# tavildar/Polar

Measured on AMD Instinct MI355X. Metric: codewords/s (N=2048 K=1024 L=32 LLR-SCL), higher is better.
Workload: dtype f64

## Files before the change

polar_amd/build.py:

```python
import os
import shutil
import subprocess
import sys

HERE = os.path.dirname(os.path.abspath(__file__))
ROOT = os.path.dirname(HERE)
CSRC = os.path.join(HERE, "csrc")
INC = os.path.join(ROOT, "include")
LIB = os.path.join(HERE, "libpolar_amd.so")
BUILD = os.path.join(HERE, "_build")
FLAGS_LIST32 = ["-mllvm", "-amdgpu-sched-strategy=max-memory-clause", "-mllvm", "-amdgpu-use-amdgpu-trackers"] + \
               os.environ.get("POLAR_LIST32_FLAGS", "").split()
FLAGS_LAT = os.environ.get("POLAR_LAT_FLAGS", "").split()
SOURCES = [("polar_kernels.hip", ["POLAR_ED_TU=0"], "", []), ("polar_kernels.hip", ["POLAR_ED_TU=1"], ".ed", []),
           ("polar_kernels.hip", ["POLAR_ED_TU=2"], ".ed32", FLAGS_LIST32), ("polar_kernels.hip", ["POLAR_ED_TU=3"], ".lat", FLAGS_LAT),
           ("polar_kernels.hip", ["POLAR_ED_TU=4"], ".list", []),
           ("polar_kernels.hip", ["POLAR_ED_TU=5"], ".headA", []), ("polar_kernels.hip", ["POLAR_ED_TU=6"], ".headB", FLAGS_LIST32),
           ("polar_kernels.hip", ["POLAR_ED_TU=7"], ".adapt", []),
           ("polar_kernels_sc.hip", [], "", []), ("polar_kernels_p1.hip", [], "", []), ("polar_channel.hip", [], "", []),
           ("polar_construct.hip", [], "", []), ("polar_kernels_mlc.hip", [], "", []), ("polar_kernels_ga.hip", [], "", []),
           ("polar_kernels_metric.hip", [], "", []), ("polar_kernels_adapt.hip", [], "", []),
           ("polar_kernels_flip.hip", [], "", [])] + \
          [(f, [], "", []) for f in ("polar_handle.cpp", "polar_decode.cpp", "polar_hostpipe.cpp", "polar_montecarlo.cpp", "polar_multi.cpp",
                                     "polar_debug.cpp", "polar_ga.cpp", "polar_bicm.cpp", "polar_list.cpp", "polar_mlc.cpp", "polar_adaptive.cpp", "polar_flip.cpp")]
TEST_HOOK_SOURCES = ("polar_montecarlo.cpp", "polar_debug.cpp")
TEST_HOOK_KERNEL_TAGS = (".ed32", ".headB")
LIB_TEST = os.path.join(HERE, "libpolar_amd_test.so")
KNOWN_DEFS = {"POLAR_MARGIN", "POLAR_SLOTHIST", "SCLAT_PROF", "POLAR_DEV_GS32", "POLAR_DEV_ONE", "POLAR_NO_FIXED_N",
              "POLAR_NO_GUARD_INT", "POLAR_NO_COLD_HINTS", "OCC", "ED_NR"}
ARCH = os.environ.get("POLAR_ARCH", "gfx950")
_flags_ok = {}


def _probe_flags(flags):
    key = tuple(flags)
    if key not in _flags_ok:
        import tempfile
        ok = list(flags)
        with tempfile.TemporaryDirectory() as d:
            src = os.path.join(d, "probe.hip")
            open(src, "w").write("#include <hip/hip_runtime.h>\n__global__ void probe_kernel() {}\n")
            pairs = [flags[i:i + 2] for i in range(0, len(flags), 2)]
            ok = []
            for pr in pairs:
                r = subprocess.run([_hipcc(), "--offload-arch=" + ARCH, "-c", src, "-o", os.path.join(d, "probe.o")] + pr,
                                   stdout=subprocess.DEVNULL, stderr=subprocess.PIPE, text=True)
                if r.returncode == 0 or "Unknown command line argument" not in r.stderr:
                    ok += pr
                else:
                    print("polar_amd.build: this compiler rejects %s (%s); building without it" %
                          (" ".join(pr), (r.stderr.strip().splitlines() or ["?"])[-1][:120]), file=sys.stderr)
        _flags_ok[key] = ok
    return _flags_ok[key]


def _hipcc():
    return shutil.which("hipcc") or "/opt/rocm/bin/hipcc"


def _torch_lib():
    try:
        import torch
        d = os.path.join(os.path.dirname(torch.__file__), "lib")
        if os.path.exists(os.path.join(d, "libamdhip64.so")):
            return d
    except Exception:
        pass
    return None


def _newer(target, deps):
    if not os.path.exists(target):
        return True
    t = os.path.getmtime(target)
    return any((not os.path.exists(d)) or os.path.getmtime(d) > t for d in deps)


def _fingerprint(cmd, files):
    import hashlib
    root = os.path.realpath(ROOT)

    def rel(x):
# ... 133 lines not shown
```

polar_amd/csrc/polar_debug.cpp:

```cpp
#include "polar_multi.h"
#include "polar_amd_debug.h"
#ifdef POLAR_TEST_HOOKS
#include "polar_head_plan.h"
hipError_t polar_r1_counts_read_ed32(unsigned long long *out);
hipError_t polar_r1_counts_read_head(unsigned long long *out);
#endif

extern "C" {

int polar_debug_weak_leaves(const polar_code_t *h) { return polar_get_weak_leaves(h); }

int polar_debug_set(polar_code_t *h, const char *key, long value) {
    if (!h || !key) return fail(POLAR_E_ARG, "NULL argument");
    polar_code::Knobs &k = h->knobs;
    const std::string s(key);
    if (s == "mode_override") { if (value < -1 || value > 2) return fail(POLAR_E_ARG, "mode_override must be -1 (none), 0, 1 or 2"); k.mode_override = (int)value; }
    else if (s == "sc_no_fold") k.sc_no_fold = value != 0;
    else if (s == "no_tables") k.no_tables = value != 0;
    else if (s == "no_head") k.no_head = value != 0;
    else if (s == "no_r1") k.no_r1 = value != 0;
    else if (s == "head_min_b") { if (value < 0) return fail(POLAR_E_ARG, "head_min_b must be >= 0 (0 = default)"); k.head_min_b = value; }
    else if (s == "no_fuse_front") k.no_fuse_front = value != 0;
    else if (s == "no_prefix") h->prefix_on = (value == 0);
    else if (s == "no_rccl") { k.no_rccl = value != 0; multi_release(h, false); }
// ... 13 lines not shown
    else if (s == "host_lanes") { if (value < 0 || value > HostPipe::kMaxLanes) return fail(POLAR_E_ARG, "host_lanes must be 0 (default) or 1 .. %d", HostPipe::kMaxLanes); k.host_lanes = value; }
    else if (s == "host_ramp") k.host_ramp = value;
    else if (s == "host_prefault") { if (value < -1 || value > 16) return fail(POLAR_E_ARG, "host_prefault must be -1 (none), 0 (default) or 1 .. 16 threads"); k.host_prefault = value; }
    else if (s == "host_threads") { if (value < 0) return fail(POLAR_E_ARG, "host_threads must be >= 0"); k.host_threads = value; }
    else if (s == "multi_grace_s") { if (value < 0) return fail(POLAR_E_ARG, "multi_grace_s must be >= 0"); k.multi_grace_s = value; }
#ifdef POLAR_TEST_HOOKS
    else if (s == "force_workers") { k.force_workers = value != 0; multi_release(h, false); }
    else if (s == "stall_device") k.stall_device = (int)value;
    else if (s == "stall_ms") { if (value < 0) return fail(POLAR_E_ARG, "stall_ms must be >= 0"); k.stall_ms = value; }
#endif
    else if (s == "multi_timeout_s") { if (value < 0) return fail(POLAR_E_ARG, "multi_timeout_s must be >= 0 (0 = no watchdog)"); k.multi_timeout_s = value; }
    else return fail(POLAR_E_ARG, "polar_debug_set: unknown key '%s'", key);
    drop_clones(h);
    return POLAR_OK;
}
void *polar_debug_scratch_ptr(polar_code_t *h) { return h ? (void *)h->d_llr_scr.p : nullptr; }
long polar_debug_get(const polar_code_t *h, const char *key) {
    if (!key) return -1;
    const std::string s(key);
    if (s == "allocs") return (long)g_allocs.load();
    if (s == "comm_inits") return (long)polar_debug_comm_inits();
    if (!h) return -1;
    if (s == "test_hooks") {
#ifdef POLAR_TEST_HOOKS
        return 1;
#else
        return 0;
#endif
    }
    if (s == "weak_leaves") return h->weak_leaves;
    if (s == "mode_override") return h->knobs.mode_override;
    if (s == "head_phi") return h->last_head_phi;
    if (s == "lat_waves") return h->last_lat_waves;
    if (s == "lane_waves") return h->last_lane_waves;
#ifdef POLAR_TEST_HOOKS
    if (s == "head_check") {
        if (!h->last_head_phi || h->last_head_b <= 0 || !h->d_head_rec.p) return -2;
        int P = 0;
        while (P < h->N && h->frozen[P]) ++P;
        const int Q = P >= 256 ? 256 : (P < 33 ? 0 : (P < 64 ? 64 : (P < 128 ? 128 : 256)));
        const HeadPlan hp = head_plan(h->frozen.data(), h->n, Q, std::min(P, Q), h->N / 2);
        if (hp.phi_h != h->last_head_phi) return -3;
        std::vector<unsigned long long> rows2((size_t)h->last_head_b * 4);
        const size_t pitch = hp.record_words() * sizeof(unsigned long long);
        if (hipMemcpy2D(rows2.data(), 32, h->d_head_rec.p + 2 * 4, pitch, 32, (size_t)h->last_head_b, hipMemcpyDeviceToHost) != hipSuccess) return -4;
        long bad = 0;
        for (long b = 0; b < h->last_head_b; ++b) {
            unsigned long long r[4];
            for (int a = 0; a < 4; ++a) r[a] = rows2[(size_t)b * 4 + a];
            bad += head_record_ok(hp, r) ? 0 : 1;
        }
        return bad;
    }
    if (s == "r1_committed" || s == "r1_discarded") {
        unsigned long long c[2] = {0, 0};
        if ((h->last_head_phi ? polar_r1_counts_read_head(c) : polar_r1_counts_read_ed32(c)) != hipSuccess) return -2;
        return (long)c[s == "r1_discarded" ? 1 : 0];
    }
#endif
    if (s == "last_rounds") return h->last_rounds;
    if (s == "last_round_max_per_device") return h->last_round_max_per_device;
    if (s == "worker_threads_started") return h->worker_threads_started;
    if (s.compare(0, 9, "round_us_") == 0) {
        if (h->round_us.empty()) return 0;
        std::vector<long> v(h->round_us);
        if (s == "round_us_count") return (long)v.size();
        if (s == "round_us_first") return v.front();
        std::sort(v.begin(), v.end());
        if (s == "round_us_min") return v.front();
        if (s == "round_us_max") return v.back();
        if (s == "round_us_median") return v[v.size() / 2];
        return -1;
    }
    if (s == "multi_poisoned") return h->multi_poisoned ? 1 : 0;
    if (s == "host_chunks") return h->hpipe ? h->hpipe->last_chunks : 0;
    if (s == "host_chunk_cw") return h->hpipe ? h->hpipe->last_chunk_cw : 0;
    if (s == "host_lanes") return h->hpipe ? h->hpipe->last_lanes : 0;
    if (s == "host_threads") return h->hpipe ? h->hpipe->last_threads : 0;
    if (s == "host_us_copy_in") return h->hpipe ? h->hpipe->us_copy_in : 0;
    if (s == "host_us_wait") return h->hpipe ? h->hpipe->us_wait : 0;
    if (s == "host_us_copy_out") return h->hpipe ? h->hpipe->us_copy_out : 0;
    if (s == "host_us_total") return h->hpipe ? h->hpipe->us_total : 0;
    return -1;
}
int polar_debug_comm_inits(void) { return g_comm_inits.load(); }

long polar_debug_fallback_rows(polar_code_t *h, uint32_t *rows, long cap) {
    if (!h || !h->fb_count) return -1;
    DevGuard dg_;
    if (ensure_device(h, dg_)) return -1;
    hipError_t e = hipStreamSynchronize((hipStream_t)h->fb_stream);
    unsigned int count = 0;
    if (e == hipSuccess) e = hipMemcpy(&count, h->fb_count, sizeof count, hipMemcpyDeviceToHost);
    if (e == hipSuccess && (long)count > h->fb_b) return -(long)hipErrorInvalidValue - 1;
    const long n = std::min<long>(count, cap);
    if (e == hipSuccess && rows && n > 0) e = hipMemcpy(rows, h->fb_list, (size_t)n * sizeof(uint32_t), hipMemcpyDeviceToHost);
    return e == hipSuccess ? (long)count : -(long)e - 1;
}

long polar_debug_ctl_words(polar_code_t *h, uint32_t *words, long cap, int marked) {
    if (!h) return -1;
    DevGuard dg_;
    if (ensure_device(h, dg_)) return -1;
    const long n = std::min<long>(h->N, cap);
    if (words && n > 0) {
        const hipError_t e = hipMemcpy(words, marked ? h->d_ctl_r1.p : h->d_ctl.p, (size_t)n * sizeof(uint32_t), hipMemcpyDeviceToHost);
        if (e != hipSuccess) return -(long)e - 1;
    }
    return h->N;
}
// ... 3 lines not shown
```

polar_amd/csrc/polar_kernels.hip:

```cpp
#include <hip/hip_runtime.h>
#include <stdint.h>
#include <type_traits>

#include "polar_kernels.h"
#include "polar_device.h"
#include "polar_edom.h"

#ifdef POLAR_PROFILE
#define PROF_DECL u64 prof_acc[32] = {0,0,0,0,0,0,0,0,0,0,0,0,0,0,0,0,0,0,0,0,0,0,0,0,0,0,0,0,0,0,0,0}; u64 prof_t = __builtin_readcyclecounter();
#define PROF(i) { u64 t_ = __builtin_readcyclecounter(); prof_acc[i] += t_ - prof_t; prof_t = t_; }
#define PROF_OUT if (lane == 0 && p.pm_out) { for (int i_ = 0; i_ < 32; ++i_) atomicAdd((u64 *)p.pm_out + i_, prof_acc[i_]); }
#define PROF_CNT(i, v) { prof_acc[i] += (u64)(v); }
#define PROF_HEAD_DECL const int prof_head_phi = p.pm_out ? (int)((const u64 *)p.pm_out)[32] : 0; const u64 prof_head_t0 = prof_t; bool prof_head_open = prof_head_phi > 0;
#define PROF_HEAD(phi_) if (prof_head_open && (phi_) >= prof_head_phi) { prof_acc[22] += __builtin_readcyclecounter() - prof_head_t0; prof_head_open = false; }
#define PROF_HEAD_END prof_acc[23] += __builtin_readcyclecounter() - prof_head_t0;
#define PROF_R1_DECL int prof_r1_left = 0; bool prof_r1_open = false; u64 prof_r1_t0 = 0; const bool prof_r1_off = p.pm_out && ((const u64 *)p.pm_out)[33] != 0; (void)prof_r1_off;
#define PROF_R1_TOP { if (prof_r1_open) { prof_acc[24] += prof_t - prof_r1_t0; prof_r1_open = false; } \
                      if (prof_r1_left > 0) { prof_r1_t0 = prof_t; prof_r1_open = true; --prof_r1_left; } }
#define PROF_R1_LEAF(ctl_, fast_) { const int rb_ = (int)((ctl_) >> 9) & 3; \
                      if (prof_r1_open) { if (!(fast_)) prof_acc[27] += 1; } \
                      else if (rb_) { if (fast_) { prof_acc[25] += 1; prof_r1_left = (1 << rb_) - 1; } else prof_acc[26] += 1; } }
#define PROF_R1_COMMIT prof_r1_left = 0;
#define PROF_R1_END if (prof_r1_open) { prof_acc[24] += __builtin_readcyclecounter() - prof_r1_t0; prof_r1_open = false; }
#else
#define PROF_R1_DECL constexpr bool prof_r1_off = false; (void)prof_r1_off;
#define PROF_R1_TOP
#define PROF_R1_LEAF(ctl_, fast_)
#define PROF_R1_COMMIT
#define PROF_R1_END
#define PROF_HEAD_DECL
#define PROF_HEAD(phi_)
#define PROF_HEAD_END
#define PROF_DECL
#define PROF(i)
#define PROF_CNT(i, v)
#define PROF_OUT
#endif

#include "polar_llr_nodes.h"

template <bool NARROW16>
__device__ __forceinline__ const double *ch_row(const PolarDecodeParams &p, size_t cw, int N) {
    if constexpr (NARROW16) {
        if (p.llr_fmt >= POLAR_LLR_F16) return reinterpret_cast<const double *>(reinterpret_cast<const uint16_t *>(p.llr) + cw * (size_t)N);
    }
    return p.llr_fmt ? reinterpret_cast<const double *>(reinterpret_cast<const float *>(p.llr) + cw * (size_t)N)
                     : p.llr + cw * (size_t)N;
}
template <bool NARROW16>
__device__ __forceinline__ double ch_narrow(const double *row, size_t i, int fmt) {
    if constexpr (NARROW16) return llr_load_narrow(row, i, fmt);
    else return (double)reinterpret_cast<const float *>(row)[i];
}
#define CH(row, i) (p.llr_fmt ? ch_narrow<CH_N16>(row, i, p.llr_fmt) : (row)[i])

#ifndef FU
#define FU 4
#endif
#ifndef POLAR_SKIP_L1
#define POLAR_SKIP_L1 1
#endif
#define POLAR_SADDR 1
#ifndef OCC
#define OCC 4
#endif
#define LANE_CTX                                   \
    const int lane = LAT ? lane_k : lane_id_opaque();    \
    const int lig = lane & (GS - 1);               \
    const int gbase = lane & ~(GS - 1);            \
    (void)lig; (void)gbase;
#if defined(POLAR_ED_TU) && POLAR_ED_TU == 4
#define POLAR_LIST_OUT 1
#define scl_decode_llr_kernel scl_decode_llr_list_kernel
#define POLAR_KPARAMS PolarListParams
#elif defined(POLAR_ED_TU) && POLAR_ED_TU == 7
#define POLAR_ADAPT_OUT 1
#define scl_decode_llr_kernel scl_decode_llr_adapt_kernel
#define POLAR_KPARAMS PolarAdaptParams
#elif defined(POLAR_ED_TU) && (POLAR_ED_TU == 5 || POLAR_ED_TU == 6)
#define POLAR_HEAD (POLAR_ED_TU == 5 ? 1 : 2)
#define scl_decode_llr_kernel scl_decode_llr_head_kernel
#define POLAR_KPARAMS PolarHeadParams
#else
#define POLAR_KPARAMS PolarDecodeParams
#endif
#ifndef POLAR_HEAD
#define POLAR_HEAD 0
#endif
#if defined(POLAR_ED_TU) && (POLAR_ED_TU == 2 || POLAR_ED_TU == 6) && !defined(POLAR_MARGIN)
#define POLAR_R1 1
#else
#define POLAR_R1 0
#endif
#if POLAR_R1 && defined(POLAR_TEST_HOOKS)
__device__ unsigned long long polar_r1_counts_dev[2];
#define R1_CNT_DECL unsigned r1_cnt_c = 0, r1_cnt_d = 0;
#define R1_CNT_COMMIT ++r1_cnt_c;
#define R1_CNT_DISCARD ++r1_cnt_d;
#define R1_CNT_OUT if (lane == 0) { atomicAdd(&polar_r1_counts_dev[0], (unsigned long long)r1_cnt_c); atomicAdd(&polar_r1_counts_dev[1], (unsigned long long)r1_cnt_d); }
#else
#define R1_CNT_DECL
#define R1_CNT_COMMIT
#define R1_CNT_DISCARD
#define R1_CNT_OUT
#endif
template <int GS, int LDS_LOG, int PIPE, bool ED, int NL = 0, int LAT = 0>
__global__ __launch_bounds__(PIPE ? 64 : 256, PIPE ? 2 : OCC) void scl_decode_llr_kernel(POLAR_KPARAMS p) {
    constexpr int WPB = PIPE ? 1 : 4;
    constexpr bool CH_N16 = !ED;
    constexpr int G = LAT ? 1 : 64 / GS;
    constexpr int EL = 64 / GS;
    constexpr int CST = LAT ? GS : 64;
#define POLAR_CL (LAT ? lig : lane)
#define POLAR_CGB (LAT ? 0 : gbase)
    constexpr int SL = 1 << LDS_LOG;
    const int lane = threadIdx.x & 63;
    const int wib = __builtin_amdgcn_readfirstlane((int)(threadIdx.x >> 6));
    const int wave_id = blockIdx.x * WPB + wib;
    const int nwaves = gridDim.x * WPB;
    const int lane_k = lane;
    (void)lane_k;
    const int lig = lane & (GS - 1);
    const int gbase = lane & ~(GS - 1);
    const int grp = LAT ? 0 : lane / GS;
    const int n = NL ? NL : p.n, N = NL ? (1 << NL) : p.N, K = p.K, L = p.L;
    const u64 gmask = (GS == 64) ? ~0ull : ((1ull << GS) - 1ull);

    extern __shared__ __attribute__((aligned(16))) unsigned char smem[];
    double *tabs = reinterpret_cast<double *>(smem);
    constexpr size_t WAVE_LDS = (size_t)(2 * SL - 1) * 64 * 8 + 128 * 8 + 128;
    unsigned char *wbase = smem + 324 * 8 + (size_t)wib * WAVE_LDS;
    double *lds_llr = reinterpret_cast<double *>(wbase);
    double *sortbuf = lds_llr + (LAT ? 0 : (size_t)(2 * SL - 1) * 64);
    unsigned char *stackv = reinterpret_cast<unsigned char *>(sortbuf + 128);
    unsigned char *srcof = stackv + 64;
    for (int i = threadIdx.x; i < 322; i += WPB * 64) tabs[i] = p.tabs[i];
    if (WPB > 1) __syncthreads();
    const Tabs tb = {tabs, tabs + 64, tabs + 64 + 129};
    u64 guard = 0;
    double gacc = __builtin_inf();
    auto FN = [&](double a, double b) -> double {
        if constexpr (ED) return f_node_e_acc(a, b, gacc); else return f_node(a, b, tb);
    };
    auto GN = [&](double a, double b, uint32_t cw_, int bi) -> double {
        if constexpr (ED) return g_node_e(a, b, cw_ << (31 - bi), tb); else return g_node(a, b, (cw_ >> bi) & 1u);
    };
    const long Bv = p.cw_count ? (long)*p.cw_count : (p.n_dev ? ((long)*p.n_dev < p.B ? (long)*p.n_dev : p.B) : p.B);

    const size_t big_elems = (N > 2 * SL) ? (size_t)(N - 2 * SL) : 0;
    double *g_llr = LAT ? nullptr : p.llr_scr + (size_t)wave_id * big_elems * 64;
    const int cwords = (N >= 128) ? (N / 32 - 2) : 0;
    double *lat_ch = reinterpret_cast<double *>(stackv + 128);
    double *lat_a = lat_ch + N;
    uint32_t *lat_w = reinterpret_cast<uint32_t *>(lat_a + (size_t)N * GS);
    uint32_t *g_cl = LAT ? lat_w : p.c_scr + (size_t)wave_id * 2 * (size_t)cwords * 64;
    uint32_t *g_cr = g_cl + (size_t)cwords * CST;
// ... 604 lines not shown
}
#elif POLAR_ED_TU == 0
hipError_t polar_launch_decode_lat_ed1(const PolarDecodeParams &p, int gs, int blocks, hipStream_t st);
hipError_t polar_launch_decode_lat(const PolarDecodeParams &p, int gs, bool ed, int blocks, hipStream_t st) {
    if (ed) return polar_launch_decode_lat_ed1(p, gs, blocks, st);
    if (gs == 2) return launch_lat<2, false>(p, blocks, st);
    return hipErrorInvalidValue;
}
size_t polar_decode_lat_lds_bytes(int N, int gs, int W) {
    return 324 * 8 + (128 * 8 + 128) + (size_t)N * 8 + (size_t)N * gs * 8 + (2 * polar_decode_cwords(N) + (size_t)3 * W) * gs * 4 + 64;
}
#endif

#if POLAR_ED_TU == 4 || POLAR_ED_TU == 7
template <int GS>
static hipError_t launch_finish(const POLAR_KPARAMS &p, int grid, hipStream_t st) {
    const int wpb = polar_decode_waves_per_block(0);
    const size_t lds = polar_decode_lds_bytes(3, 0);
    hipLaunchKernelGGL((scl_decode_llr_kernel<GS, 3, 0, false>), dim3(grid / wpb), dim3(64 * wpb), lds, st, p);
    return hipGetLastError();
}
static hipError_t launch_finish_gs(const POLAR_KPARAMS &p, int gs, int grid, hipStream_t st) {
    switch (gs) {
        case 1: return launch_finish<1>(p, grid, st);
        case 2: return launch_finish<2>(p, grid, st);
        case 4: return launch_finish<4>(p, grid, st);
        case 8: return launch_finish<8>(p, grid, st);
        case 16: return launch_finish<16>(p, grid, st);
        case 32: return launch_finish<32>(p, grid, st);
        case 64: return launch_finish<64>(p, grid, st);
        default: return hipErrorInvalidValue;
    }
}
#if POLAR_ED_TU == 4
hipError_t polar_launch_decode_llr_list(const PolarListParams &p, int gs, int grid, hipStream_t st) {
    if (!p.list_cand || grid < 4 || (grid & 3)) return hipErrorInvalidValue;
    return launch_finish_gs(p, gs, grid, st);
}
#else
hipError_t polar_launch_decode_llr_adapt(const PolarAdaptParams &p, int gs, int grid, hipStream_t st) {
    if (!p.out || !p.ad_retry || grid < 4 || (grid & 3)) return hipErrorInvalidValue;
    return launch_finish_gs(p, gs, grid, st);
}
#endif
#elif POLAR_ED_TU == 5
hipError_t polar_launch_decode_head_export(const PolarHeadParams &p, int grid, hipStream_t st) {
    if (!p.head_rec || p.L != 4 || p.head_phi <= 0 || p.head_phi >= p.N || grid < 4 || (grid & 3)) return hipErrorInvalidValue;
    hipLaunchKernelGGL((scl_decode_llr_kernel<4, 3, 0, true>), dim3(grid / 4), dim3(256), polar_decode_lds_bytes(3, 0), st, p);
    return hipGetLastError();
}
#elif POLAR_ED_TU == 6
#ifdef POLAR_TEST_HOOKS
static hipError_t r1_counts_zero(hipStream_t st) {
    static const unsigned long long z[2] = {0, 0};
    return hipMemcpyToSymbolAsync(HIP_SYMBOL(polar_r1_counts_dev), z, sizeof z, 0, hipMemcpyHostToDevice, st);
}
hipError_t polar_r1_counts_read_head(unsigned long long *out) { return hipMemcpyFromSymbol(out, HIP_SYMBOL(polar_r1_counts_dev), 2 * sizeof(unsigned long long)); }
#endif
hipError_t polar_launch_decode_head_import(const PolarHeadParams &p, int grid, hipStream_t st) {
#ifdef POLAR_TEST_HOOKS
    if (hipError_t e = r1_counts_zero(st)) return e;
#endif
    if (!p.head_rec || p.L < 17 || p.L > 32 || p.head_phi <= 0 || p.head_phi >= p.N || grid < 4 || (grid & 3)) return hipErrorInvalidValue;
    const size_t lds = polar_decode_lds_bytes(3, 0);
#ifndef POLAR_NO_FIXED_N
    if (p.n == 11) hipLaunchKernelGGL((scl_decode_llr_kernel<32, 3, 0, true, 11>), dim3(grid / 4), dim3(256), lds, st, p);
    else if (p.n == 10) hipLaunchKernelGGL((scl_decode_llr_kernel<32, 3, 0, true, 10>), dim3(grid / 4), dim3(256), lds, st, p);
    else
#endif
    hipLaunchKernelGGL((scl_decode_llr_kernel<32, 3, 0, true>), dim3(grid / 4), dim3(256), lds, st, p);
    return hipGetLastError();
}
#elif POLAR_ED_TU == 2
#ifdef POLAR_TEST_HOOKS
hipError_t polar_r1_counts_read_ed32(unsigned long long *out) { return hipMemcpyFromSymbol(out, HIP_SYMBOL(polar_r1_counts_dev), 2 * sizeof(unsigned long long)); }
#endif
hipError_t polar_launch_decode_llr_ed1_gs32(const PolarDecodeParams &p, int lds_log, int pipe, int grid, hipStream_t st) {
#ifdef POLAR_TEST_HOOKS
    {
        static const unsigned long long z[2] = {0, 0};
        if (hipError_t e = hipMemcpyToSymbolAsync(HIP_SYMBOL(polar_r1_counts_dev), z, sizeof z, 0, hipMemcpyHostToDevice, st)) return e;
    }
#endif
    return launch_gs<32, true>(p, lds_log, pipe, grid, st);
}
#elif POLAR_ED_TU == 1
hipError_t polar_launch_decode_llr_ed1_gs32(const PolarDecodeParams &p, int lds_log, int pipe, int grid, hipStream_t st);
hipError_t polar_launch_decode_llr_ed1(const PolarDecodeParams &p, int gs, int lds_log, int pipe, int grid, hipStream_t st) {
    switch (gs) {
#ifndef POLAR_DEV_GS32
        case 4: return launch_gs<4, true>(p, lds_log, pipe, grid, st);
        case 8: return launch_gs<8, true>(p, lds_log, pipe, grid, st);
        case 16: return launch_gs<16, true>(p, lds_log, pipe, grid, st);
        case 64: return launch_gs<64, true>(p, lds_log, pipe, grid, st);
#endif
        case 32: return polar_launch_decode_llr_ed1_gs32(p, lds_log, pipe, grid, st);
        default: return hipErrorInvalidValue;
    }
}
#elif POLAR_ED_TU == 0
hipError_t polar_launch_decode_llr_ed0(const PolarDecodeParams &p, int gs, int lds_log, int pipe, int grid, hipStream_t st) {
    switch (gs) {
        case 1: return launch_gs<1, false>(p, lds_log, pipe, grid, st);
#ifndef POLAR_DEV_GS32
        case 2: return launch_gs<2, false>(p, lds_log, pipe, grid, st);
        case 4: return launch_gs<4, false>(p, lds_log, pipe, grid, st);
        case 8: return launch_gs<8, false>(p, lds_log, pipe, grid, st);
        case 16: return launch_gs<16, false>(p, lds_log, pipe, grid, st);
        case 64: return launch_gs<64, false>(p, lds_log, pipe, grid, st);
#endif
        case 32: return launch_gs<32, false>(p, lds_log, pipe, grid, st);
        default: return hipErrorInvalidValue;
    }
}
hipError_t polar_launch_decode_llr(const PolarDecodeParams &p, int gs, int lds_log, int pipe, int grid, bool ed, hipStream_t st) {
    return ed ? polar_launch_decode_llr_ed1(p, gs, lds_log, pipe, grid, st) : polar_launch_decode_llr_ed0(p, gs, lds_log, pipe, grid, st);
}
#endif
```

polar_amd/csrc/polar_scl_leaf.inc:

```
            if (zb) {
                const int Z = 1 << zb;
                LANE_CTX
                auto block4 = [&](double v0, double v1, double v2, double v3) {
                    double lf[4] = {0, 0, 0, 0};
                    if (active) {
                        double a0, a1;
                        FN2(v0, v2, v1, v3, a0, a1);
                        const double b0 = GN(v0, v2, 0u, 0), b1 = GN(v1, v3, 0u, 0);
                        FN2(a0, a1, b0, b1, lf[0], lf[2]);
                        lf[1] = GN(a0, a1, 0u, 0); lf[3] = GN(b0, b1, 0u, 0);
                    }
                    if constexpr (LAT && ED) {
                        bool ng[4]; double alz[4], sneg[4], spos[4];
                        leaf_terms_ed_block<4>(lf, actw, tb, ng, alz, sneg, spos);
#pragma unroll
                        for (int i = 0; i < 4; ++i)
                            if (active) pm += ng[i] ? spos[i] : sneg[i];
                    } else {
#pragma unroll
                    for (int i = 0; i < 4; ++i) {
                        bool ng; double alz, sneg, spos;
                        leaf_terms<ED>(lf[i], active, actw, tb, ng, alz, sneg, spos);
                        if (active) pm += ng ? spos : sneg;
                    }
// ... 36 lines not shown
                phi += Z - 1;
                continue;
            }
            LANE_CTX
            const u64 below = (1ull << lig) - 1ull;
            const bool frozen = (ctl & 1u) != 0;
            unsigned ubit = 0;
            if (frozen) {
                bool ng; double alz, sneg, spos;
                if constexpr (LAT && ED) {
                    const double lf1[1] = {leaf}; bool ng1[1]; double al1[1], sn1[1], sp1[1];
                    leaf_terms_ed_block<1>(lf1, actw, tb, ng1, al1, sn1, sp1);
                    ng = ng1[0]; alz = al1[0]; sneg = sn1[0]; spos = sp1[0];
                } else leaf_terms<ED>(leaf, active, actw, tb, ng, alz, sneg, spos);
                if (active) pm += ng ? spos : sneg;
            } else {
                const u64 actm = LAT ? (actw & gmask) : ((actw >> gbase) & gmask);
                const int nact = __popcll(actm);
                const int rho = (2 * nact < L) ? 2 * nact : L;
                bool lneg; double al;
                double gm = -__builtin_inf(), bl = __builtin_inf();
                double sneg, spos;
                if constexpr (LAT && ED) {
                    const double lf1[1] = {leaf}; bool ng1[1]; double al1[1], sn1[1], sp1[1];
                    leaf_terms_ed_block<1>(lf1, actw, tb, ng1, al1, sn1, sp1);
                    lneg = ng1[0]; al = al1[0]; sneg = sn1[0]; spos = sp1[0];
                } else leaf_terms<ED>(leaf, active, actw, tb, lneg, al, sneg, spos);
                if constexpr (ED) {
                    if (POLAR_UNLIKELY2(ctl & 0x100u)) guard |= __ballot(active && fabs(leaf) > 0.99999999 && fabs(leaf) <= 1.0);
                }
                if (active) {
                    gm = pm + sneg;
                    bl = (pm + al) * 0.99999999999909050530;
                }
                bool fast;
                {
                    unsigned gh = active ? (unsigned)__double2hiint(gm) : 0u;
                    unsigned bh = active ? (unsigned)__double2hiint(bl) : 0xFFFFFFFFu;
                    group_max_min_u32<GS>(gh, bh);
                    if constexpr (LAT) {
                        fast = (nact == 0) || (nact == L && ((__builtin_amdgcn_uicmp(gh, bh, 36) | ~group_result_rows<GS>()) == ~0ull));
                    } else {
                    const u64 m_ok = __builtin_amdgcn_sicmp(nact, 0, 32) | (__builtin_amdgcn_sicmp(nact, L, 32) & __builtin_amdgcn_uicmp(gh, bh, 36));
                    fast = ((m_ok | ~group_result_rows<GS>()) == ~0ull);
                    }
                }
                double gmax = 0.0;
                if (!fast) {
                    gmax = group_reduce<GS, true>(gm, lane);
                    const double bmin = group_reduce<GS, false>(bl, lane);
                    fast = wave_all((nact == 0) || (nact == L && gmax < bmin));
                }
                PROF_CNT(8, 1)
                PROF_R1_LEAF(ctl, fast)
                PROF(16)
                if (fast) {
                    PROF_CNT(9, 1)
#ifdef POLAR_MARGIN
                    {
                        const double gx = group_reduce<GS, true>(active ? gm : -__builtin_inf(), lane);
                        const double bx = group_reduce<GS, false>(active ? pm + spos : __builtin_inf(), lane);
                        if (nact == L) mingap = __builtin_fmin(mingap, bx - gx);
                    }
#endif
                    if (active) {
                        ubit = lneg ? 1u : 0u;
                        pm = gm;
                        hword |= ubit << (t & 31);
                    }
                    PROF(17)
#if POLAR_R1
                    if constexpr (ED && !LAT && GS == 32) {
                    if ((ctl & 0x600u) && !prof_r1_off) {
                        PROF_CNT(29, 1)
                        const uint32_t ctl_r1 = ctlp[phi + 4 < N ? phi + 4 : 0];
                        const double *yq = lds_llr + (size_t)1 * 64 + lane, *xq = lds_llr + (size_t)3 * 64 + lane;
                        double lf[3] = {0.0, 0.0, 0.0};
                        if (active) {
                            const double y0 = yq[0], y1 = yq[64], x0 = xq[0], x1 = xq[64], x2 = xq[128], x3 = xq[192];
                            auto gss = [&](double a_, double b_) { return g_node_e(a_, b_, (unsigned)(__double2hiint(a_) ^ __double2hiint(b_)), tb); };
                            const double z0 = gss(x0, x2), z1 = gss(x1, x3);
                            lf[0] = gss(y0, y1);
                            lf[1] = FN(z0, z1);
                            lf[2] = gss(z0, z1);
                        }
                        double pmq = pm;
                        u64 m_lt = ~0ull, m_one = __builtin_amdgcn_fcmp(fabs(leaf), 1.0, 1);
                        uint32_t uq = 0;
#pragma unroll
                        for (int i_ = 0; i_ < 3; ++i_) {
                            bool ng1; double al1, sn1, sp1;
                            leaf_terms<ED>(lf[i_], active, actw, tb, ng1, al1, sn1, sp1);
                            const double gq = pmq + sn1, bq = (pmq + al1) * 0.99999999999909050530;
                            unsigned gh_ = active ? (unsigned)__double2hiint(gq) : 0u, bh_ = active ? (unsigned)__double2hiint(bq) : 0xFFFFFFFFu;
                            group_max_min_u32<GS>(gh_, bh_);
                            m_lt &= __builtin_amdgcn_uicmp(gh_, bh_, 36);
                            m_one |= __builtin_amdgcn_fcmp(fabs(lf[i_]), 1.0, 1);
                            pmq = gq;
                            uq |= (ng1 ? 1u : 0u) << i_;
                        }
                        const u64 m_okq = __builtin_amdgcn_sicmp(nact, 0, 32) | (__builtin_amdgcn_sicmp(nact, L, 32) & m_lt);
                        const bool pass = ((m_okq | ~group_result_rows<GS>()) == ~0ull) && (m_one & actw) == 0;
                        if (pass) {
                            PROF_CNT(30, 1)
                            PROF_CNT(8, 3)
                            PROF_CNT(9, 3)
                            PROF_R1_COMMIT
                            const uint32_t u1 = uq & 1u, u2 = (uq >> 1) & 1u, u3 = uq >> 2;
                            if (active) {
                                pm = pmq;
                                hword |= (u1 << ((t + 1) & 31)) | (u2 << ((t + 2) & 31)) | (u3 << ((t + 3) & 31));
                            }
                            const uint32_t X = (ubit ^ u1 ^ u2 ^ u3) | ((u1 ^ u3) << 1) | ((u2 ^ u3) << 2) | (u3 << 3);
                            const int nu = phi >> 2;
                            if ((nu & 1) == 0) {
                                if (active) clsmall = (clsmall & ~(0xFull << 4)) | ((u64)X << 4);
                            } else {
                                update_c(4, X, nu);
                            }
                            wave_mem_fence();
                            t += 3;
                            phi += 3;
                            ctl_next = ctl_r1;
                            r1_done = true;
                            R1_CNT_COMMIT
                        } else {
                            R1_CNT_DISCARD
                        }
                        PROF(28)
                    }
                    }
#endif
                } else {
                double pf0 = __builtin_nan(""), pf1 = __builtin_nan("");
                if (active) {
                    pf0 = -(pm + (lneg ? spos : sneg));
                    pf1 = -(pm + (lneg ? sneg : spos));
                }
                bool c0 = active, c1 = active;
                const bool need = (2 * nact > L);
                const bool full = (nact == L);
                if (POLAR_LIKELY2(!wave_any(need && !full))) {
                    const bool goodbit = lneg;
                    const double mg = goodbit ? -pf1 : -pf0;
                    const double mb = goodbit ? -pf0 : -pf1;
                    const bool cbad = active && full && !(bl > gmax);
                    const u64 cbm = __ballot(cbad);
                    bool sg, sbd;
                    if constexpr (GS == 32) {
                        const u64 actm64 = actw;
                        const u64 gbm = __ballot(goodbit);
                        u64 surv = 0;
                        PROF_CNT(10, 1)
                        PROF_CNT(11, __popcll(cbm))
                        for (u64 mi = cbm; mi; mi &= mi - 1) {
                            const int l_ = __builtin_ctzll(mi);
                            const double s_mb = readlane_d(mb, l_);
                            const u64 grp = 0xFFFFFFFFull << (l_ & 32);
                            const u64 blw = ((1ull << l_) - 1ull) & grp;
                            const u64 self_first = ~gbm & (1ull << l_);
                            const u64 lt_g = __builtin_amdgcn_fcmp(mg, s_mb, 4), eq_g = __builtin_amdgcn_fcmp(mg, s_mb, 1);
                            const u64 lt_b = __builtin_amdgcn_fcmp(mb, s_mb, 4), eq_b = __builtin_amdgcn_fcmp(mb, s_mb, 1);
                            const int r = __popcll((lt_g | (eq_g & (blw | self_first))) & grp & actm64) +
                                          __popcll((lt_b | (eq_b & blw)) & grp & cbm);
                            if (r < L) surv |= 1ull << l_;
                        }
                        PROF(18)
                        int k0 = __popcll(surv & 0xFFFFFFFFull), k1 = __popcll(surv >> 32);
                        u64 alive = actm64;
                        const unsigned khi = (unsigned)__double2hiint(mg) + 1u, klo = (unsigned)__double2loint(mg);
                        auto peel = [&](u64 e, int &k) {
                            const int ne = __popcll(e);
                            if (ne == 0) { k = 0; return; }
                            if (ne <= k) { alive &= ~e; k -= ne; return; }
                            for (; k > 0; --k) {
                                int best = -1; unsigned blo = 0;
                                for (u64 q = e; q; q &= q - 1) {
                                    const int l_ = __builtin_ctzll(q);
                                    const unsigned lo_ = (unsigned)__builtin_amdgcn_readlane((int)klo, l_);
                                    if (best < 0 || lo_ >= blo) { best = l_; blo = lo_; }
                                }
                                e &= ~(1ull << best);
                                alive &= ~(1ull << best);
                            }
                        };
// ... 116 lines not shown
                    sp += __popcll(km);
                    wave_mem_fence();
                    if (both) {
                        int lp = stackv[gbase + sp - 1 - __popcll(bm & below)];
                        srcof[gbase + lp] = (unsigned char)lig;
                    }
                    sp -= __popcll(bm);
                    wave_mem_fence();
                }
                const int src = srcof[lane];
                const bool is_clone = (src != lig);
                PROF(20)
                double pm_new = c0 ? -pf0 : -pf1;
                ubit = c0 ? 0u : 1u;
                if (wave_any(is_clone)) {
                    const int sl = gbase + src;
                    double pm1 = shfl_d(-pf1, sl);
                    u64 a0 = shfl_u64(pL.lo, sl), a1 = shfl_u64(pL.hi, sl);
                    u64 b0 = shfl_u64(pC.lo, sl), b1 = shfl_u64(pC.hi, sl);
                    u64 cs = shfl_u64(clsmall, sl);
                    uint32_t hw = __shfl(hword, sl, 64);
                    int og = __shfl(origin, sl, 64);
                    if (is_clone) {
                        pm_new = pm1; ubit = 1u;
                        pL.lo = a0; pL.hi = a1; pC.lo = b0; pC.hi = b1;
                        clsmall = cs; hword = hw; origin = og;
                    }
                    if constexpr (LAT) {
                        if ((n >= 3) ? ((phi & 1) == 0) : lat_yv) {
                            const double y0_ = shfl_d(lat_y0, sl), y1_ = shfl_d(lat_y1, sl);
                            if (is_clone) { lat_y0 = y0_; lat_y1 = y1_; }
                        }
                        if (n >= 3 && (phi & 3) < 2) {
                            double x_[4];
#pragma unroll
                            for (int k = 0; k < 4; ++k) x_[k] = shfl_d(lat_x[k], sl);
                            if (is_clone) {
#pragma unroll
                                for (int k = 0; k < 4; ++k) lat_x[k] = x_[k];
                            }
                        }
                    }
                }
                active = (active && !kill) || is_clone;
                actw = __ballot(active);
                if (active) {
                    pm = pm_new;
                    hword |= ubit << (t & 31);
                } else {
                    pm = 0.0;
                }
                PROF(21)
                }
                if (POLAR_UNLIKELY2((t & 31) == 31)) {
                    const int w = (int)(t >> 5);
                    if (active) {
                        g_hist[(size_t)w * CST + POLAR_CL] = hword;
                        g_horg[(size_t)w * CST + POLAR_CL] = (uint32_t)origin;
                        origin = lig;
                        hword = 0;
                    }
                    wave_mem_fence();
                }
                ++t;
            }

            PROF(frozen ? 5 : 6)
#if POLAR_R1
            if (r1_done) {
            } else
#endif
            if ((phi & 1) == 0) {
                if (active) clsmall = (clsmall & ~2ull) | ((u64)ubit << 1);
            } else {
                update_c(1, ubit, phi);
            }
            PROF(7)
```

Measured before the change: 1.118 million.

## Extend rate-1 leaf shortcut to ranked leaves and chain into octets

```diff
diff --git a/polar_amd/build.py b/polar_amd/build.py
--- a/polar_amd/build.py
+++ b/polar_amd/build.py
@@ -27,7 +27,7 @@
 TEST_HOOK_KERNEL_TAGS = (".ed32", ".headB")
 LIB_TEST = os.path.join(HERE, "libpolar_amd_test.so")
 KNOWN_DEFS = {"POLAR_MARGIN", "POLAR_SLOTHIST", "SCLAT_PROF", "POLAR_DEV_GS32", "POLAR_DEV_ONE", "POLAR_NO_FIXED_N",
-              "POLAR_NO_GUARD_INT", "POLAR_NO_COLD_HINTS", "OCC", "ED_NR"}
+              "POLAR_NO_GUARD_INT", "POLAR_NO_COLD_HINTS", "OCC", "ED_NR", "POLAR_R1_RANK", "POLAR_R1_CHAIN"}
 ARCH = os.environ.get("POLAR_ARCH", "gfx950")
 _flags_ok = {}
 
diff --git a/polar_amd/csrc/polar_debug.cpp b/polar_amd/csrc/polar_debug.cpp
--- a/polar_amd/csrc/polar_debug.cpp
+++ b/polar_amd/csrc/polar_debug.cpp
@@ -89,10 +89,14 @@
         }
         return bad;
     }
-    if (s == "r1_committed" || s == "r1_discarded") {
-        unsigned long long c[2] = {0, 0};
-        if ((h->last_head_phi ? polar_r1_counts_read_head(c) : polar_r1_counts_read_ed32(c)) != hipSuccess) return -2;
-        return (long)c[s == "r1_discarded" ? 1 : 0];
+    if (s.compare(0, 3, "r1_") == 0) {
+        static const char *const names[6] = {"r1_committed", "r1_discarded", "r1_rank_tried", "r1_rank_committed", "r1_chain_tried", "r1_chain_committed"};
+        for (int i = 0; i < 6; ++i) {
+            if (s != names[i]) continue;
+            unsigned long long c[6] = {0, 0, 0, 0, 0, 0};
+            if ((h->last_head_phi ? polar_r1_counts_read_head(c) : polar_r1_counts_read_ed32(c)) != hipSuccess) return -2;
+            return (long)c[i];
+        }
     }
 #endif
     if (s == "last_rounds") return h->last_rounds;
diff --git a/polar_amd/csrc/polar_kernels.hip b/polar_amd/csrc/polar_kernels.hip
--- a/polar_amd/csrc/polar_kernels.hip
+++ b/polar_amd/csrc/polar_kernels.hip
@@ -7,26 +7,33 @@
 #include "polar_edom.h"
 
 #ifdef POLAR_PROFILE
-#define PROF_DECL u64 prof_acc[32] = {0,0,0,0,0,0,0,0,0,0,0,0,0,0,0,0,0,0,0,0,0,0,0,0,0,0,0,0,0,0,0,0}; u64 prof_t = __builtin_readcyclecounter();
+#define PROF_DECL u64 prof_acc[40] = {0,0,0,0,0,0,0,0,0,0,0,0,0,0,0,0,0,0,0,0,0,0,0,0,0,0,0,0,0,0,0,0,0,0,0,0,0,0,0,0}; u64 prof_t = __builtin_readcyclecounter();
 #define PROF(i) { u64 t_ = __builtin_readcyclecounter(); prof_acc[i] += t_ - prof_t; prof_t = t_; }
-#define PROF_OUT if (lane == 0 && p.pm_out) { for (int i_ = 0; i_ < 32; ++i_) atomicAdd((u64 *)p.pm_out + i_, prof_acc[i_]); }
+#define PROF_OUT if (lane == 0 && p.pm_out) { for (int i_ = 0; i_ < 40; ++i_) atomicAdd((u64 *)p.pm_out + (i_ < 32 ? i_ : i_ + 2), prof_acc[i_]); }
 #define PROF_CNT(i, v) { prof_acc[i] += (u64)(v); }
 #define PROF_HEAD_DECL const int prof_head_phi = p.pm_out ? (int)((const u64 *)p.pm_out)[32] : 0; const u64 prof_head_t0 = prof_t; bool prof_head_open = prof_head_phi > 0;
 #define PROF_HEAD(phi_) if (prof_head_open && (phi_) >= prof_head_phi) { prof_acc[22] += __builtin_readcyclecounter() - prof_head_t0; prof_head_open = false; }
 #define PROF_HEAD_END prof_acc[23] += __builtin_readcyclecounter() - prof_head_t0;
-#define PROF_R1_DECL int prof_r1_left = 0; bool prof_r1_open = false; u64 prof_r1_t0 = 0; const bool prof_r1_off = p.pm_out && ((const u64 *)p.pm_out)[33] != 0; (void)prof_r1_off;
-#define PROF_R1_TOP { if (prof_r1_open) { prof_acc[24] += prof_t - prof_r1_t0; prof_r1_open = false; } \
+#define PROF_R1_DECL int prof_r1_left = 0, prof_r1_slot = 24; bool prof_r1_open = false; u64 prof_r1_t0 = 0; \
+                     const unsigned prof_r1_sw = p.pm_out ? (unsigned)((const u64 *)p.pm_out)[33] : 0u; \
+                     const bool prof_r1_off = (prof_r1_sw & 1u) != 0, prof_rank_off = (prof_r1_sw & 2u) != 0, prof_chain_off = (prof_r1_sw & 4u) != 0; \
+                     (void)prof_r1_off; (void)prof_rank_off; (void)prof_chain_off;
+#define PROF_R1_ADD(d_) { if (prof_r1_slot == 24) prof_acc[24] += (d_); else if (prof_r1_slot == 32) prof_acc[32] += (d_); else prof_acc[34] += (d_); }
+#define PROF_R1_TOP { if (prof_r1_open) { PROF_R1_ADD(prof_t - prof_r1_t0) prof_r1_open = false; } \
                       if (prof_r1_left > 0) { prof_r1_t0 = prof_t; prof_r1_open = true; --prof_r1_left; } }
-#define PROF_R1_LEAF(ctl_, fast_) { const int rb_ = (int)((ctl_) >> 9) & 3; \
-                      if (prof_r1_open) { if (!(fast_)) prof_acc[27] += 1; } \
-                      else if (rb_) { if (fast_) { prof_acc[25] += 1; prof_r1_left = (1 << rb_) - 1; } else prof_acc[26] += 1; } }
+#define PROF_R1_LEAF(ctl_, fast_, full_) { const int rb_ = (int)((ctl_) >> 9) & 3; \
+                      if (prof_r1_open) { if (!(fast_) && prof_r1_slot == 24) prof_acc[27] += 1; } \
+                      else if (rb_) { if (fast_) { prof_acc[25] += 1; prof_r1_left = (1 << rb_) - 1; prof_r1_slot = 24; } \
+                                      else { prof_acc[26] += 1; if (full_) { prof_acc[33] += 1; prof_r1_left = 3; prof_r1_slot = 32; } } } }
 #define PROF_R1_COMMIT prof_r1_left = 0;
-#define PROF_R1_END if (prof_r1_open) { prof_acc[24] += __builtin_readcyclecounter() - prof_r1_t0; prof_r1_open = false; }
+#define PROF_R1_OCTET(open_) if (open_) { prof_acc[35] += 1; prof_r1_left = 1; prof_r1_slot = 34; }
+#define PROF_R1_END if (prof_r1_open) { PROF_R1_ADD(__builtin_readcyclecounter() - prof_r1_t0) prof_r1_open = false; }
 #else
-#define PROF_R1_DECL constexpr bool prof_r1_off = false; (void)prof_r1_off;
+#define PROF_R1_DECL constexpr bool prof_r1_off = false, prof_rank_off = false, prof_chain_off = false; (void)prof_r1_off; (void)prof_rank_off; (void)prof_chain_off;
 #define PROF_R1_TOP
-#define PROF_R1_LEAF(ctl_, fast_)
+#define PROF_R1_LEAF(ctl_, fast_, full_)
 #define PROF_R1_COMMIT
+#define PROF_R1_OCTET(open_)
 #define PROF_R1_END
 #define PROF_HEAD_DECL
 #define PROF_HEAD(phi_)
@@ -92,16 +99,20 @@
 #else
 #define POLAR_R1 0
 #endif
+#ifndef POLAR_R1_RANK
+#define POLAR_R1_RANK 1
+#endif
+#ifndef POLAR_R1_CHAIN
+#define POLAR_R1_CHAIN 1
+#endif
 #if POLAR_R1 && defined(POLAR_TEST_HOOKS)
-__device__ unsigned long long polar_r1_counts_dev[2];
-#define R1_CNT_DECL unsigned r1_cnt_c = 0, r1_cnt_d = 0;
-#define R1_CNT_COMMIT ++r1_cnt_c;
-#define R1_CNT_DISCARD ++r1_cnt_d;
-#define R1_CNT_OUT if (lane == 0) { atomicAdd(&polar_r1_counts_dev[0], (unsigned long long)r1_cnt_c); atomicAdd(&polar_r1_counts_dev[1], (unsigned long long)r1_cnt_d); }
+__device__ unsigned long long polar_r1_counts_dev[6];
+#define R1_CNT_DECL unsigned r1_cnt[6] = {0, 0, 0, 0, 0, 0};
+#define R1_CNT(i_) ++r1_cnt[i_];
+#define R1_CNT_OUT if (lane == 0) { for (int i_ = 0; i_ < 6; ++i_) atomicAdd(&polar_r1_counts_dev[i_], (unsigned long long)r1_cnt[i_]); }
 #else
 #define R1_CNT_DECL
-#define R1_CNT_COMMIT
-#define R1_CNT_DISCARD
+#define R1_CNT(i_)
 #define R1_CNT_OUT
 #endif
 template <int GS, int LDS_LOG, int PIPE, bool ED, int NL = 0, int LAT = 0>
@@ -812,10 +823,10 @@
 #elif POLAR_ED_TU == 6
 #ifdef POLAR_TEST_HOOKS
 static hipError_t r1_counts_zero(hipStream_t st) {
-    static const unsigned long long z[2] = {0, 0};
+    static const unsigned long long z[6] = {0, 0, 0, 0, 0, 0};
     return hipMemcpyToSymbolAsync(HIP_SYMBOL(polar_r1_counts_dev), z, sizeof z, 0, hipMemcpyHostToDevice, st);
 }
-hipError_t polar_r1_counts_read_head(unsigned long long *out) { return hipMemcpyFromSymbol(out, HIP_SYMBOL(polar_r1_counts_dev), 2 * sizeof(unsigned long long)); }
+hipError_t polar_r1_counts_read_head(unsigned long long *out) { return hipMemcpyFromSymbol(out, HIP_SYMBOL(polar_r1_counts_dev), 6 * sizeof(unsigned long long)); }
 #endif
 hipError_t polar_launch_decode_head_import(const PolarHeadParams &p, int grid, hipStream_t st) {
 #ifdef POLAR_TEST_HOOKS
@@ -833,12 +844,12 @@
 }
 #elif POLAR_ED_TU == 2
 #ifdef POLAR_TEST_HOOKS
-hipError_t polar_r1_counts_read_ed32(unsigned long long *out) { return hipMemcpyFromSymbol(out, HIP_SYMBOL(polar_r1_counts_dev), 2 * sizeof(unsigned long long)); }
+hipError_t polar_r1_counts_read_ed32(unsigned long long *out) { return hipMemcpyFromSymbol(out, HIP_SYMBOL(polar_r1_counts_dev), 6 * sizeof(unsigned long long)); }
 #endif
 hipError_t polar_launch_decode_llr_ed1_gs32(const PolarDecodeParams &p, int lds_log, int pipe, int grid, hipStream_t st) {
 #ifdef POLAR_TEST_HOOKS
     {
-        static const unsigned long long z[2] = {0, 0};
+        static const unsigned long long z[6] = {0, 0, 0, 0, 0, 0};
         if (hipError_t e = hipMemcpyToSymbolAsync(HIP_SYMBOL(polar_r1_counts_dev), z, sizeof z, 0, hipMemcpyHostToDevice, st)) return e;
     }
 #endif
diff --git a/polar_amd/csrc/polar_scl_leaf.inc b/polar_amd/csrc/polar_scl_leaf.inc
--- a/polar_amd/csrc/polar_scl_leaf.inc
+++ b/polar_amd/csrc/polar_scl_leaf.inc
@@ -112,7 +112,7 @@
                     fast = wave_all((nact == 0) || (nact == L && gmax < bmin));
                 }
                 PROF_CNT(8, 1)
-                PROF_R1_LEAF(ctl, fast)
+                PROF_R1_LEAF(ctl, fast, ((__builtin_amdgcn_sicmp(nact, 0, 32) | __builtin_amdgcn_sicmp(nact, L, 32)) == ~0ull))
                 PROF(16)
                 if (fast) {
                     PROF_CNT(9, 1)
@@ -129,68 +129,6 @@
                         hword |= ubit << (t & 31);
                     }
                     PROF(17)
-#if POLAR_R1
-                    if constexpr (ED && !LAT && GS == 32) {
-                    if ((ctl & 0x600u) && !prof_r1_off) {
-                        PROF_CNT(29, 1)
-                        const uint32_t ctl_r1 = ctlp[phi + 4 < N ? phi + 4 : 0];
-                        const double *yq = lds_llr + (size_t)1 * 64 + lane, *xq = lds_llr + (size_t)3 * 64 + lane;
-                        double lf[3] = {0.0, 0.0, 0.0};
-                        if (active) {
-                            const double y0 = yq[0], y1 = yq[64], x0 = xq[0], x1 = xq[64], x2 = xq[128], x3 = xq[192];
-                            auto gss = [&](double a_, double b_) { return g_node_e(a_, b_, (unsigned)(__double2hiint(a_) ^ __double2hiint(b_)), tb); };
-                            const double z0 = gss(x0, x2), z1 = gss(x1, x3);
-                            lf[0] = gss(y0, y1);
-                            lf[1] = FN(z0, z1);
-                            lf[2] = gss(z0, z1);
-                        }
-                        double pmq = pm;
-                        u64 m_lt = ~0ull, m_one = __builtin_amdgcn_fcmp(fabs(leaf), 1.0, 1);
-                        uint32_t uq = 0;
-#pragma unroll
-                        for (int i_ = 0; i_ < 3; ++i_) {
-                            bool ng1; double al1, sn1, sp1;
-                            leaf_terms<ED>(lf[i_], active, actw, tb, ng1, al1, sn1, sp1);
-                            const double gq = pmq + sn1, bq = (pmq + al1) * 0.99999999999909050530;
-                            unsigned gh_ = active ? (unsigned)__double2hiint(gq) : 0u, bh_ = active ? (unsigned)__double2hiint(bq) : 0xFFFFFFFFu;
-                            group_max_min_u32<GS>(gh_, bh_);
-                            m_lt &= __builtin_amdgcn_uicmp(gh_, bh_, 36);
-                            m_one |= __builtin_amdgcn_fcmp(fabs(lf[i_]), 1.0, 1);
-                            pmq = gq;
-                            uq |= (ng1 ? 1u : 0u) << i_;
-                        }
-                        const u64 m_okq = __builtin_amdgcn_sicmp(nact, 0, 32) | (__builtin_amdgcn_sicmp(nact, L, 32) & m_lt);
-                        const bool pass = ((m_okq | ~group_result_rows<GS>()) == ~0ull) && (m_one & actw) == 0;
-                        if (pass) {
-                            PROF_CNT(30, 1)
-                            PROF_CNT(8, 3)
-                            PROF_CNT(9, 3)
-                            PROF_R1_COMMIT
-                            const uint32_t u1 = uq & 1u, u2 = (uq >> 1) & 1u, u3 = uq >> 2;
-                            if (active) {
-                                pm = pmq;
-                                hword |= (u1 << ((t + 1) & 31)) | (u2 << ((t + 2) & 31)) | (u3 << ((t + 3) & 31));
-                            }
-                            const uint32_t X = (ubit ^ u1 ^ u2 ^ u3) | ((u1 ^ u3) << 1) | ((u2 ^ u3) << 2) | (u3 << 3);
-                            const int nu = phi >> 2;
-                            if ((nu & 1) == 0) {
-                                if (active) clsmall = (clsmall & ~(0xFull << 4)) | ((u64)X << 4);
-                            } else {
-                                update_c(4, X, nu);
-                            }
-                            wave_mem_fence();
-                            t += 3;
-                            phi += 3;
-                            ctl_next = ctl_r1;
-                            r1_done = true;
-                            R1_CNT_COMMIT
-                        } else {
-                            R1_CNT_DISCARD
-                        }
-                        PROF(28)
-                    }
-                    }
-#endif
                 } else {
                 double pf0 = __builtin_nan(""), pf1 = __builtin_nan("");
                 if (active) {
@@ -413,6 +351,135 @@
                 }
                 PROF(21)
                 }
+#if POLAR_R1
+                if constexpr (ED && !LAT && GS == 32) {
+                bool r1_go = false;
+                if ((ctl & 0x600u) && !prof_r1_off) {
+                    r1_go = fast;
+#if POLAR_R1_RANK
+                    if (!fast && !prof_rank_off) r1_go = ((__builtin_amdgcn_sicmp(nact, 0, 32) | __builtin_amdgcn_sicmp(nact, L, 32)) == ~0ull);
+#endif
+                }
+                if (r1_go) {
+                    PROF_CNT(29, 1)
+                    if (!fast) { PROF_CNT(36, 1) R1_CNT(2) }
+                    const uint32_t ctl_r1 = ctlp[phi + 4 < N ? phi + 4 : 0];
+                    double lf[3] = {0.0, 0.0, 0.0};
+                    double gq = gacc;
+                    if (active) {
+                        const double *yq = lds_llr + (size_t)1 * 64 + gbase + pL.get(1), *xq = lds_llr + (size_t)3 * 64 + gbase + pL.get(2);
+                        const double y0 = yq[0], y1 = yq[64], x0 = xq[0], x1 = xq[64], x2 = xq[128], x3 = xq[192];
+                        const unsigned s0 = ubit << 31;
+                        lf[0] = g_node_e(y0, y1, s0, tb);
+                        const unsigned s1 = (unsigned)__double2hiint(lf[0]);
+                        const double z0 = g_node_e(x0, x2, s0 ^ s1, tb), z1 = g_node_e(x1, x3, s1, tb);
+                        lf[1] = f_node_e_acc(z0, z1, gq);
+                        lf[2] = g_node_e(z0, z1, (unsigned)__double2hiint(lf[1]), tb);
+                    }
+                    double pmq = pm;
+                    auto tests = [&](const auto &lv, u64 m_one, uint32_t &uq) -> bool {
+                        constexpr int CNT = (int)(sizeof(lv) / sizeof(double));
+                        u64 m_lt = ~0ull;
+                        uq = 0;
+#pragma unroll
+                        for (int i_ = 0; i_ < CNT; ++i_) {
+                            bool ng1; double al1, sn1, sp1;
+                            leaf_terms<ED>(lv[i_], active, actw, tb, ng1, al1, sn1, sp1);
+                            const double gq_ = pmq + sn1, bq_ = (pmq + al1) * 0.99999999999909050530;
+                            unsigned gh_ = active ? (unsigned)__double2hiint(gq_) : 0u, bh_ = active ? (unsigned)__double2hiint(bq_) : 0xFFFFFFFFu;
+                            group_max_min_u32<GS>(gh_, bh_);
+                            m_lt &= __builtin_amdgcn_uicmp(gh_, bh_, 36);
+                            m_one |= __builtin_amdgcn_fcmp(fabs(lv[i_]), 1.0, 1);
+                            pmq = gq_;
+                            uq |= (ng1 ? 1u : 0u) << i_;
+                        }
+                        const u64 m_okq = __builtin_amdgcn_sicmp(nact, 0, 32) | (__builtin_amdgcn_sicmp(nact, L, 32) & m_lt);
+                        return ((m_okq | ~group_result_rows<GS>()) == ~0ull) && (m_one & actw) == 0;
+                    };
+                    uint32_t uq;
+                    const bool pass = tests(lf, fast ? __builtin_amdgcn_fcmp(fabs(leaf), 1.0, 1) : 0ull, uq);
+                    if (pass) {
+                        PROF_CNT(30, 1)
+                        PROF_CNT(8, 3)
+                        PROF_CNT(9, 3)
+                        PROF_R1_COMMIT
+                        if (fast) { R1_CNT(0) } else { PROF_CNT(37, 1) R1_CNT(3) }
+                        const uint32_t u1 = uq & 1u, u2 = (uq >> 1) & 1u, u3 = uq >> 2;
+                        if (active) {
+                            pm = pmq;
+                            hword |= (u1 << ((t + 1) & 31)) | (u2 << ((t + 2) & 31)) | (u3 << ((t + 3) & 31));
+                        }
+                        gacc = gq;
+                        uint32_t X = (ubit ^ u1 ^ u2 ^ u3) | ((u1 ^ u3) << 1) | ((u2 ^ u3) << 2) | (u3 << 3);
+                        int Sx = 4, adv = 3;
+                        uint32_t ctl_after = ctl_r1;
+                        bool octet_open = (ctl & 0x600u) == 0x600u;
+                        (void)octet_open;
+#if POLAR_R1_CHAIN
+                        if constexpr (LDS_LOG >= 3) {
+                        if ((ctl & 0x600u) == 0x600u && !prof_chain_off) {
+                            PROF_CNT(38, 1)
+                            R1_CNT(4)
+                            const uint32_t ctl_r2 = ctlp[phi + 8 < N ? phi + 8 : 0];
+                            double lc[4] = {0.0, 0.0, 0.0, 0.0};
+                            double gq2 = gq;
+                            if (active) {
+                                const double *wq = lds_llr + (size_t)7 * 64 + gbase + pL.get(3);
+                                double wa[4], wb[4], w[4];
+#pragma unroll
+                                for (int j = 0; j < 4; ++j) { wa[j] = wq[(size_t)j * 64]; wb[j] = wq[(size_t)(j + 4) * 64]; }
+#pragma unroll
+                                for (int j = 0; j < 4; ++j) w[j] = g_node_e(wa[j], wb[j], X << (31 - j), tb);
+                                const double y0 = f_node_e_acc(w[0], w[2], gq2), y1 = f_node_e_acc(w[1], w[3], gq2);
+                                lc[0] = f_node_e_acc(y0, y1, gq2);
+                                const unsigned s0 = (unsigned)__double2hiint(lc[0]);
+                                lc[1] = g_node_e(y0, y1, s0, tb);
+                                const unsigned s1 = (unsigned)__double2hiint(lc[1]);
+                                const double z0 = g_node_e(w[0], w[2], s0 ^ s1, tb), z1 = g_node_e(w[1], w[3], s1, tb);
+                                lc[2] = f_node_e_acc(z0, z1, gq2);
+                                lc[3] = g_node_e(z0, z1, (unsigned)__double2hiint(lc[2]), tb);
+                            }
+                            uint32_t uc;
+                            if (tests(lc, 0ull, uc)) {
+                                PROF_CNT(39, 1)
+                                PROF_CNT(8, 4)
+                                PROF_CNT(9, 4)
+                                R1_CNT(5)
+                                R1_CNT(0)
+                                const uint32_t u4 = uc & 1u, u5 = (uc >> 1) & 1u, u6 = (uc >> 2) & 1u, u7 = uc >> 3;
+                                if (active) {
+                                    pm = pmq;
+                                    hword |= (u4 << ((t + 4) & 31)) | (u5 << ((t + 5) & 31)) | (u6 << ((t + 6) & 31)) | (u7 << ((t + 7) & 31));
+                                }
+                                gacc = gq2;
+                                const uint32_t X2 = (u4 ^ u5 ^ u6 ^ u7) | ((u5 ^ u7) << 1) | ((u6 ^ u7) << 2) | (u7 << 3);
+                                X = (X ^ X2) | (X2 << 4);
+                                Sx = 8; adv = 7;
+                                ctl_after = ctl_r2;
+                                octet_open = false;
+                            }
+                        }
+                        }
+#endif
+                        PROF_R1_OCTET(octet_open)
+                        const int nu = phi >> (Sx == 8 ? 3 : 2);
+                        if ((nu & 1) == 0) {
+                            if (active) clsmall = (Sx == 8) ? ((clsmall & ~(0xFFull << 8)) | ((u64)X << 8)) : ((clsmall & ~(0xFull << 4)) | ((u64)X << 4));
+                        } else {
+                            update_c(Sx, X, nu);
+                        }
+                        wave_mem_fence();
+                        t += adv;
+                        phi += adv;
+                        ctl_next = ctl_after;
+                        r1_done = true;
+                    } else {
+                        if (fast) { R1_CNT(1) }
+                    }
+                    PROF(28)
+                }
+                }
+#endif
                 if (POLAR_UNLIKELY2((t & 31) == 31)) {
                     const int w = (int)(t >> 5);
                     if (active) {
```

Result: faster. 1.135 million (median of 6 runs) (+1.6%).
